# zhu-xlab/PFST

Measured on AMD Instinct MI355X. Metric: PFST train-step images/s on 1024² IRRG tiles, higher is better.
Workload: dtype f32 (f16x3 split MFMA: two scaled fp16 pieces per operand, three products, fp32 accumulate); 1 GPU; pfst_pots_irrg2vaih_irrg_deeplabv3plus_r50-d8; global_batch=8, per_gpu_batch=8, tile=1024x1024x3, num_classes=6, parallelism=dp1, weights=seeded random init, conv_math=f16x3

## Files before the change

### pfst_amd/csrc/conv_epilogue.h

```cpp
#pragma once
#include <type_traits>
#include <utility>
#include "common.h"
#ifndef PFST_BNB_LOAD_AUX
#define PFST_BNB_LOAD_AUX 0
#endif
#include "../../include/pfst_hip.h"

typedef float pfst_f32x16 __attribute__((ext_vector_type(16)));

__device__ __forceinline__ bool src_coord(int o, int t, int a, int b, int c0, int div, int lim, int& s) {
  const int v = o * a + t * b + c0;
  const int odd = v & (div - 1);
  s = v >> (div >> 1);
  return (odd == 0) & (s >= 0) & (s < lim);
}

template <int... Is, class F>
__device__ __forceinline__ void static_for_seq(std::integer_sequence<int, Is...>, F&& f) {
  (f(std::integral_constant<int, Is>()), ...);
}
template <int N, class F>
__device__ __forceinline__ void static_for(F&& f) {
  static_for_seq(std::make_integer_sequence<int, N>(), static_cast<F&&>(f));
}

typedef pfst_bnb_fuse_t PfstBnbArgs;

template <int CTRL>
__device__ __forceinline__ float lane_xchg(float v) {
  if (CTRL == 0) return __builtin_bit_cast(float, __builtin_amdgcn_ds_swizzle(__builtin_bit_cast(int, v), 0x401F));
  return __builtin_bit_cast(float, __builtin_amdgcn_update_dpp(0, __builtin_bit_cast(int, v), CTRL, 0xF, 0xF, true));
}
template <int OP>
__device__ __forceinline__ float lane_combine(float a, float b) {
  return OP == 0 ? a + b : (OP == 1 ? fminf(a, b) : fmaxf(a, b));
}
template <int H, int CTRL, int OP = 0>
__device__ __forceinline__ void butterfly_step(float* a, bool upper) {
#pragma unroll
  for (int k = 0; k < H; ++k) {
    const float send = upper ? a[k] : a[k + H];
    const float keep = upper ? a[k + H] : a[k];
    a[k] = lane_combine<OP>(keep, lane_xchg<CTRL>(send));
  }
}
template <int NV, int OP = 0>
__device__ __forceinline__ float half_wave_transpose_reduce(float (&a)[NV], int l31) {
  static_assert(NV == 32 || NV == 16, "one value per accumulator row of a 64- or 32-row wave tile");
  if (NV == 32) {
    butterfly_step<16, 0, OP>(a, (l31 & 16) != 0);
  } else {
#pragma unroll
    for (int k = 0; k < 16; ++k) a[k] = lane_combine<OP>(a[k], lane_xchg<0>(a[k]));
  }
  butterfly_step<8, 0x140, OP>(a, (l31 & 8) != 0);
  butterfly_step<4, 0x141, OP>(a, (l31 & 4) != 0);
  butterfly_step<2, 0x4E, OP>(a, (l31 & 2) != 0);
  butterfly_step<1, 0xB1, OP>(a, (l31 & 1) != 0);
  return a[0];
}
template <int NV>
__device__ __forceinline__ float half_wave_transpose_sum(float (&a)[NV], int l31) { return half_wave_transpose_reduce<NV, 0>(a, l31); }

constexpr int PFST_ROWSUM_LDS_FLOATS = 64 * 20;
__device__ __forceinline__ void wave_lds_phase_fence() {
  __builtin_amdgcn_fence(__ATOMIC_RELEASE, "wavefront");
  __builtin_amdgcn_wave_barrier();
  __builtin_amdgcn_fence(__ATOMIC_ACQUIRE, "wavefront");
}

__device__ __forceinline__ float half_wave_rowsum_lds(const float (&v)[16], float* __restrict__ ws, int lane) {
  float4* wr = reinterpret_cast<float4*>(ws + lane * 20);
  wave_lds_phase_fence();
  wr[0] = make_float4(v[0], v[1], v[2], v[3]);
  wr[1] = make_float4(v[4], v[5], v[6], v[7]);
  wr[2] = make_float4(v[8], v[9], v[10], v[11]);
  wr[3] = make_float4(v[12], v[13], v[14], v[15]);
  wave_lds_phase_fence();
  const int l31 = lane & 31;
  const float* rd = ws + ((lane & 32) + (l31 >> 4)) * 20 + (l31 & 15);
  float s = 0.f;
#pragma unroll
  for (int i = 0; i < 16; ++i) s += rd[i * 40];
  return s + lane_xchg<0>(s);
}

template <int TM, int TN, int WAVES_N, int BN, int BNB = 0, bool LDSRED = false>
__device__ __forceinline__ void conv_epilogue(pfst_f32x16 (&acc)[TM][TN], float* __restrict__ out, const float* __restrict__ bias,
                                              float* __restrict__ stats, int stats_T, int accumulate, int M, int P, int m0, int p0,
                                              int wm0, int wn0, int bx, int n, int wid, int lane, const PfstBnbArgs& bnb = PfstBnbArgs(),
                                              float* __restrict__ lds = nullptr, const float* __restrict__ gsrc = nullptr,
                                              const unsigned long long* __restrict__ gmask = nullptr, float* __restrict__ stats_mm = nullptr,
                                              bool nt_store = false) {
  const int l31 = lane & 31, lh = lane >> 5;
  if (BNB == 0 && stats) {
    const int gx = (P + BN - 1) / BN;
    const int slot = (n * gx + bx) * WAVES_N + (wid % WAVES_N);
    if constexpr (LDSRED) {
      float* ws = lds + wid * PFST_ROWSUM_LDS_FLOATS;
#pragma unroll
      for (int i = 0; i < TM; ++i) {
        float sv[16], sq[16];
#pragma unroll
        for (int r = 0; r < 16; ++r) {
          float a = 0.f, b = 0.f;
#pragma unroll
          for (int j = 0; j < TN; ++j) {
            const int pp = p0 + wn0 + j * 32 + l31;
            const float v = pp < P ? acc[i][j][r] : 0.f;
            a += v;
            b = fmaf(v, v, b);
          }
          sv[r] = a;
          sq[r] = b;
        }
        const float ts = half_wave_rowsum_lds(sv, ws, lane);
        const float tq = half_wave_rowsum_lds(sq, ws, lane);
        const int r = l31 & 15;
        const int m = m0 + wm0 + i * 32 + (r & 3) + 8 * (r >> 2) + 4 * lh;
        if (l31 < 16 && m < M) reinterpret_cast<float2*>(stats)[(i64)m * stats_T + slot] = make_float2(ts, tq);
      }
    } else {
    constexpr int NV = TM * 16;
    float sv[NV], sq[NV];
#pragma unroll
    for (int i = 0; i < TM; ++i) {
#pragma unroll
      for (int r = 0; r < 16; ++r) {
        float a = 0.f, b = 0.f;
#pragma unroll
        for (int j = 0; j < TN; ++j) {
          const int pp = p0 + wn0 + j * 32 + l31;
          const float v = pp < P ? acc[i][j][r] : 0.f;
          a += v;
          b = fmaf(v, v, b);
        }
        sv[i * 16 + r] = a;
        sq[i * 16 + r] = b;
      }
    }
    const float ts = half_wave_transpose_sum<NV>(sv, l31);
    const float tq = half_wave_transpose_sum<NV>(sq, l31);
    const int e = l31 & (NV - 1), r = e & 15;
    const int m = m0 + wm0 + (e >> 4) * 32 + (r & 3) + 8 * (r >> 2) + 4 * lh;
    if (l31 < NV && m < M) {
      float2* dst = reinterpret_cast<float2*>(stats) + ((i64)m * stats_T + slot);
      *dst = make_float2(ts, tq);
    }
    if (stats_mm) {
      const float inf = __builtin_inff();
#pragma unroll
      for (int i = 0; i < TM; ++i) {
#pragma unroll
        for (int rr = 0; rr < 16; ++rr) {
          float lo = inf, hi = -inf;
#pragma unroll
          for (int j = 0; j < TN; ++j) {
            const int pp = p0 + wn0 + j * 32 + l31;
            const float v = acc[i][j][rr];
            lo = pp < P ? fminf(lo, v) : lo;
            hi = pp < P ? fmaxf(hi, v) : hi;
          }
          sv[i * 16 + rr] = lo;
          sq[i * 16 + rr] = hi;
        }
      }
      const float tlo = half_wave_transpose_reduce<NV, 1>(sv, l31);
      const float thi = half_wave_transpose_reduce<NV, 2>(sq, l31);
      if (l31 < NV && m < M) reinterpret_cast<float2*>(stats_mm)[(i64)m * stats_T + slot] = make_float2(tlo, thi);
    }
    }
  }
  if (BNB != 0 || (!bias && m0 + wm0 + TM * 32 <= M)) {
    constexpr unsigned OOB = 0x80000000u;
    const __amdgpu_buffer_rsrc_t rsrc = __builtin_amdgcn_make_buffer_rsrc(out, 0, M * P * 4, 0x00020000);
    unsigned voff[TN];
#pragma unroll
    for (int j = 0; j < TN; ++j) {
      const int pp = p0 + wn0 + j * 32 + l31;
      voff[j] = pp < P ? 4u * ((unsigned)pp + 4u * (unsigned)lh * (unsigned)P) : OOB;
    }
    const int row0 = m0 + wm0;
    const bool gated = gsrc != nullptr;
    static_assert(TN <= 2, "the gate words are shared by the column blocks of a 64-pixel wave tile");
    const __amdgpu_buffer_rsrc_t grs = __builtin_amdgcn_make_buffer_rsrc(const_cast<float*>(gated ? gsrc : out), 0, M * P * 4, 0x00020000);
    const __amdgpu_buffer_rsrc_t mrs =
        __builtin_amdgcn_make_buffer_rsrc(const_cast<unsigned long long*>(gmask), 0, gated ? M * (P >> 6) * 8 : 0, 0x00020000);
    const int gpp = p0 + wn0 + l31, gbit = (gpp & 255) >> 2;
    const unsigned mvoff = 8u * (unsigned)((gpp >> 8) * 4 + (gpp & 3)) + 4u * (unsigned)(gbit >> 5) + 32u * (unsigned)lh * (unsigned)(P >> 6);
    auto load_gate = [&](int i, int (&gw)[16]) {
#pragma unroll
      for (int r = 0; r < 16; ++r)
        gw[r] = gated ? __builtin_amdgcn_raw_buffer_load_b32(mrs, mvoff, 8 * (P >> 6) * (row0 + i * 32 + (r & 3) + 8 * (r >> 2)), 0) : 0;
    };
    auto load_addend = [&](int i, int j, const int (&gw)[16], float (&old)[16]) {
#pragma unroll
      for (int r = 0; r < 16; ++r)
        old[r] = __builtin_bit_cast(float, __builtin_amdgcn_raw_buffer_load_b32(grs, voff[j], 4 * P * (row0 + i * 32 + (r & 3) + 8 * (r >> 2)), 0));
      if (gated) {
        const unsigned sh = (unsigned)((gbit & 31) + 8 * j);
#pragma unroll
        for (int r = 0; r < 16; ++r)
          old[r] = __builtin_bit_cast(float, __builtin_bit_cast(int, old[r]) & __builtin_amdgcn_sbfe(gw[r], sh, 1u));
      }
    };
    if (BNB && (accumulate || gated)) {
#pragma unroll
      for (int i = 0; i < TM; ++i) {
        int gw[16];
        load_gate(i, gw);
#pragma unroll
        for (int j = 0; j < TN; ++j) {
          float old[16];
          load_addend(i, j, gw, old);
#pragma unroll
          for (int r = 0; r < 16; ++r) acc[i][j][r] += old[r];
        }
      }
    }
    if (BNB || !(accumulate || gated)) {
      auto store_all = [&](auto aux_c) {
        constexpr int AUX = decltype(aux_c)::value;
#pragma unroll
        for (int i = 0; i < TM; ++i)
#pragma unroll
          for (int j = 0; j < TN; ++j) {
#pragma unroll
            for (int r = 0; r < 16; ++r) {
              const float v = acc[i][j][r];
#ifdef PFST_DIAG_NO_STORE
              if (v != 1.2345e-30f) continue;
#endif
              __builtin_amdgcn_raw_buffer_store_b32(__builtin_bit_cast(unsigned, v), rsrc, voff[j],
                                                    4 * P * (row0 + i * 32 + (r & 3) + 8 * (r >> 2)), AUX);
            }
          }
      };
#ifdef PFST_BNB_NT_STORE
      if (nt_store) store_all(std::integral_constant<int, 2>());
#else
      if (BNB == 0 && nt_store) store_all(std::integral_constant<int, 2>());
#endif
      else store_all(std::integral_constant<int, 0>());
    } else {
#pragma unroll
      for (int i = 0; i < TM; ++i) {
        int gw[16];
        load_gate(i, gw);
#pragma unroll
        for (int j = 0; j < TN; ++j) {
          float old[16];
          load_addend(i, j, gw, old);
#pragma unroll
          for (int r = 0; r < 16; ++r)
          {
            const float v = acc[i][j][r] + old[r];
            __builtin_amdgcn_raw_buffer_store_b32(__builtin_bit_cast(unsigned, v), rsrc, voff[j],
                                                  4 * P * (row0 + i * 32 + (r & 3) + 8 * (r >> 2)), 0);
          }
        }
      }
    }
    if (BNB) {
      const __amdgpu_buffer_rsrc_t xr = __builtin_amdgcn_make_buffer_rsrc(const_cast<float*>(bnb.x) + (i64)n * bnb.x_bs, 0, M * P * 4, 0x00020000);
      const __amdgpu_buffer_rsrc_t yr = __builtin_amdgcn_make_buffer_rsrc(const_cast<float*>(bnb.y ? bnb.y + (i64)n * bnb.y_bs : bnb.x), 0,
                                                                          M * P * 4, 0x00020000);
      const __amdgpu_buffer_rsrc_t cr = __builtin_amdgcn_make_buffer_rsrc(const_cast<float*>(bnb.coef), 0, M * 16, 0x00020000);
      constexpr bool gate_x = BNB == 1, gate_y = BNB == 2, gate_m = BNB == 4;
      const __amdgpu_buffer_rsrc_t ymr = __builtin_amdgcn_make_buffer_rsrc(
          const_cast<unsigned long long*>(gate_m ? bnb.y_mask + (i64)n * M * (P >> 6) : nullptr), 0, gate_m ? M * (P >> 6) * 8 : 0, 0x00020000);
      const unsigned cvoff = 64u * (unsigned)lh + 8u;
      const int gxp = (P + BN - 1) / BN;
      const int slot = (n * gxp + bx) * WAVES_N + (wid % WAVES_N);
#pragma unroll
      for (int i = 0; i < TM; ++i) {
        float sv[16], sq[16];
        int yw[gate_m ? 16 : 1];
        if constexpr (gate_m) {
#pragma unroll
          for (int r = 0; r < 16; ++r)
            yw[r] = __builtin_amdgcn_raw_buffer_load_b32(ymr, mvoff, 8 * (P >> 6) * (row0 + i * 32 + (r & 3) + 8 * (r >> 2)), 0);
        }
#pragma unroll
        for (int r = 0; r < 16; ++r) {
          const int row = row0 + i * 32 + (r & 3) + 8 * (r >> 2);
          float sc = 0.f, sh = 0.f;
          if (gate_x) {
            const float2 c2 = __builtin_bit_cast(float2, __builtin_amdgcn_raw_buffer_load_b64(cr, cvoff, 16 * row, 0));
            sc = c2.x; sh = c2.y;
          }
          float a = 0.f, b = 0.f;
#pragma unroll
          for (int j = 0; j < TN; ++j) {
            const float xv = __builtin_bit_cast(float, __builtin_amdgcn_raw_buffer_load_b32(xr, voff[j], 4 * P * row, PFST_BNB_LOAD_AUX));
            float dz = voff[j] != OOB ? acc[i][j][r] : 0.f;
            if (gate_y) {
              const float yv = __builtin_bit_cast(float, __builtin_amdgcn_raw_buffer_load_b32(yr, voff[j], 4 * P * row, PFST_BNB_LOAD_AUX));
              dz = yv > 0.f ? dz : 0.f;
            } else if (gate_x) {
              dz = __fmaf_rn(xv, sc, sh) > 0.f ? dz : 0.f;
            } else if constexpr (gate_m) {
              dz = __builtin_bit_cast(float, __builtin_bit_cast(int, dz) & __builtin_amdgcn_sbfe(yw[r], (unsigned)((gbit & 31) + 8 * j), 1u));
            }
            a += dz;
            b = fmaf(dz, xv, b);
          }
          sv[r] = a;
          sq[r] = b;
          if ((r & 3) == 3) __builtin_amdgcn_sched_barrier(0);
        }
        float* ws = lds + wid * PFST_ROWSUM_LDS_FLOATS;
        const float ts = LDSRED ? half_wave_rowsum_lds(sv, ws, lane) : half_wave_transpose_sum<16>(sv, l31);
        const float tq = LDSRED ? half_wave_rowsum_lds(sq, ws, lane) : half_wave_transpose_sum<16>(sq, l31);
        const int r = l31 & 15;
        const int m = row0 + i * 32 + (r & 3) + 8 * (r >> 2) + 4 * lh;
        if (l31 < 16) reinterpret_cast<float2*>(bnb.partials)[(i64)m * stats_T + slot] = make_float2(ts, tq);
      }
    }
    return;
  }
#pragma unroll
  for (int i = 0; i < TM; ++i) {
#pragma unroll
    for (int j = 0; j < TN; ++j) {
      const int pp = p0 + wn0 + j * 32 + l31;
#pragma unroll
      for (int r = 0; r < 16; ++r) {
        const int m = m0 + wm0 + i * 32 + (r & 3) + 8 * (r >> 2) + 4 * lh;
        if (m < M && pp < P) {
          float v = acc[i][j][r];
          if (bias) v += bias[m];
          const i64 idx = (i64)m * P + pp;
          if (accumulate) v += out[idx];
          out[idx] = v;
        }
      }
    }
  }
}
```

### pfst_amd/csrc/conv_f16x3.hip

```cpp
#include "conv_epilogue.h"
#include "amax.h"
#include "wgrad_launch.h"
#include "weight_jobs.h"
#include <math.h>
#include <stdlib.h>
#include <type_traits>
#include <utility>
#include "../../include/pfst_hip.h"

typedef _Float16 f16x8 __attribute__((ext_vector_type(8)));
typedef float f32x4 __attribute__((ext_vector_type(4)));

namespace {

constexpr int BN = 128;
constexpr int NP = 2;

__global__ __launch_bounds__(256) void absmax_kernel(const float* __restrict__ x, i64 n, i64 plane_stride, int slot_stride,
                                                     float* __restrict__ slots) {
  const float* p = x + (i64)blockIdx.y * plane_stride;
  float m = 0.f;
  const i64 n4 = (((uintptr_t)p & 15) == 0) ? n / 4 : 0;
  for (i64 i = (i64)blockIdx.x * blockDim.x + threadIdx.x; i < n4; i += (i64)gridDim.x * blockDim.x) {
    const float4 v = reinterpret_cast<const float4*>(p)[i];
// ... 269 lines not shown
        voff2 = tap_voff(0);
      } else {
        voff2 = OOB;
      }
    }
  };

  const int eb = amax_exponent(amax_read(in_amax));
  const float sb = __builtin_bit_cast(float, __builtin_amdgcn_readfirstlane(__builtin_bit_cast(int, scale_of(eb))));
  int ea = 0, ea_y = -1;

  auto prologue = [&](int lin) {
    ld_lin = lin;
    set_load_side(lin);
    tap2 = sidx2 = 0;
    voff2 = tap_voff(0);
    static_for<8 * TPT>([&](auto vc) { load_b(vc, std::integral_constant<int, 0>(), voff2, 0); });
    static_for<NA>([&](auto vc) { load_a(vc, std::integral_constant<int, 0>(), 0); });
    advance();
#pragma unroll
    for (int v = 0; v < NA; ++v) As[(v / (NA / 2)) * TILE_A + tid + NT * (v % (NA / 2))] = areg[0][v];
#pragma unroll
    for (int t = 0; t < TPT; ++t) {
      uint4 ph, pl;
      if constexpr (BNL) {
        const float2* cf = reinterpret_cast<const float2*>(bnl_s) + (t + bt) * 16 + kh * 8;
#pragma unroll
        for (int i = 0; i < 8; ++i) breg[0][t][i] = fmaxf(__fmaf_rn(breg[0][t][i], cf[i].x, cf[i].y), 0.f);
      }
      if constexpr (BPACK) unpack8_f16(breg[0][t], ph, pl);
      else split8_f16(breg[0][t], sb, ph, pl);
      Bs[(t + bt) * TILE_B + (0 * 2 + kh) * BN + pix] = ph;
      Bs[(t + bt) * TILE_B + (1 * 2 + kh) * BN + pix] = pl;
    }
    {
      const int soff = sidx2 * chan_step, a_soff = (tap2 * spt + sidx2) * 2 * a_tile;
      static_for<8 * TPT>([&](auto vc) { load_b(vc, std::integral_constant<int, 1>(), voff2, soff); });
      static_for<NA>([&](auto vc) { load_a(vc, std::integral_constant<int, 1>(), a_soff); });
    }
    advance();
    __syncthreads();
  };

  const int l15 = lane & 15, lq = lane >> 4;
  const int a_frag = (lq >> 1) * TILE_A + (lq & 1) * BM + wm0 + l15;
  const int b_frag = (lq >> 1) * TILE_B + (lq & 1) * BN + wn0 + l15;

  const int l31 = lane & 31, lh = lane >> 5;
  auto step32 = [&](auto setn_c, int k) {
    constexpr int SETN = decltype(setn_c)::value, SETL = SETN ^ 1;
    constexpr int CUR = SETL * PAIR_CHUNKS, NXT = SETN * PAIR_CHUNKS;
    f16x8 af[2][TMW][NP], bf[2][2][NP];
    auto rd_a = [&](int t, int i, int pl) { af[t][i][pl] = __builtin_bit_cast(f16x8, As[CUR + t * TILE_A + (pl * 2 + lh) * BM + wm0 + i * 32 + l31]); };
    auto rd_b = [&](int t, int j, int pl) { bf[t][j][pl] = __builtin_bit_cast(f16x8, Bs[CUR + t * TILE_B + (pl * 2 + lh) * BN + wn0 + j * 32 + l31]); };
    constexpr int RG = 2 + TMW;
    auto read_frag = [&](auto rc) {
      constexpr int r = decltype(rc)::value, grp = r / RG, e = r % RG, t = grp & 1, pa = grp < 2 ? 1 : 0, pb = grp < 2 ? 0 : 1;
      if constexpr (e == 0) rd_a(t, 0, pa);
      else if constexpr (e == 1) rd_b(t, 0, pb);
      else if constexpr (e == 2) rd_b(t, 1, pb);
      else rd_a(t, 1, pa);
    };
    const int soff2 = sidx2 * chan_step;
    const int a_soff2 = (tap2 * spt + sidx2) * 2 * a_tile;
    constexpr int PRE = TMW == 2 ? RG : 2 * RG;
    static_for<PRE>([&](auto rc) { read_frag(rc); });
    __builtin_amdgcn_sched_barrier(0);
    SplitF16 s0, s1;
    uint4 cfr[BNL ? 4 : 1];
    const int cf_at = BNL ? sidx1 * 16 + bt * 8 + kh * 4 : 0;
    auto filler = [&](auto sc) {
      constexpr int m = decltype(sc)::value;
      if constexpr (m < 8) {
        if constexpr (TPT == 2) {
          load_b(std::integral_constant<int, 2 * m>(), std::integral_constant<int, SETL>(), voff2, soff2);
          load_b(std::integral_constant<int, 2 * m + 1>(), std::integral_constant<int, SETL>(), voff2, soff2);
        } else {
          load_b(std::integral_constant<int, m>(), std::integral_constant<int, SETL>(), voff2, soff2);
        }
      }
      if constexpr (m >= 8 && m < 8 + NA) As[NXT + ((m - 8) / (NA / 2)) * TILE_A + tid + NT * ((m - 8) % (NA / 2))] = areg[SETN][m - 8];
      if constexpr (BNL && m >= 8 && m < 12) cfr[m - 8] = bnl_s[cf_at + (m - 8)];
      if constexpr (m >= 12) {
        constexpr int SPS = 2 * TPT;
        static_for<SPS>([&](auto kc) {
          constexpr int kk = (m - 12) * SPS + decltype(kc)::value;
          if constexpr (BPACK) {
            if constexpr (kk < 8) unpack_op_f16<kk>(breg[SETN][0], s0);
            else if constexpr (kk < 16 && TPT == 2) unpack_op_f16<kk - 8>(breg[SETN][TPT - 1], s1);
          } else {
            if constexpr (BNL && kk < 24 && kk % 6 < 2) {
              constexpr int e = 2 * (kk / 6) + kk % 6;
              const uint4 c2 = cfr[e >> 1];
              const float sc = __builtin_bit_cast(float, (e & 1) ? c2.z : c2.x), sh = __builtin_bit_cast(float, (e & 1) ? c2.w : c2.y);
              breg[SETN][0][e] = fmaxf(__fmaf_rn(breg[SETN][0][e], sc, sh), 0.f);
            }
            if constexpr (kk < 24) split_op_f16<kk>(breg[SETN][0], sb, s0);
            else split_op_f16<kk - 24>(breg[SETN][TPT - 1], sb, s1);
          }
        });
      }
      if constexpr (m >= 12 && m < 12 + NA) load_a(std::integral_constant<int, m - 12>(), std::integral_constant<int, SETL>(), a_soff2);
      if constexpr (m == 18 && TPT == 2) {
        Bs[NXT + (0 * 2 + kh) * BN + pix] = make_uint4(s0.h[0], s0.h[1], s0.h[2], s0.h[3]);
        Bs[NXT + (1 * 2 + kh) * BN + pix] = make_uint4(s0.l[0], s0.l[1], s0.l[2], s0.l[3]);
      }
      if constexpr (m == 23 && TPT == 2) {
        Bs[NXT + TILE_B + (0 * 2 + kh) * BN + pix] = make_uint4(s1.h[0], s1.h[1], s1.h[2], s1.h[3]);
        Bs[NXT + TILE_B + (1 * 2 + kh) * BN + pix] = make_uint4(s1.l[0], s1.l[1], s1.l[2], s1.l[3]);
      }
      if constexpr (m == 23 && TPT == 1) {
        Bs[NXT + bt * TILE_B + (0 * 2 + kh) * BN + pix] = make_uint4(s0.h[0], s0.h[1], s0.h[2], s0.h[3]);
        Bs[NXT + bt * TILE_B + (1 * 2 + kh) * BN + pix] = make_uint4(s0.l[0], s0.l[1], s0.l[2], s0.l[3]);
      }
    };
    static_for<12 * TMW>([&](auto mc) {
      constexpr int m = decltype(mc)::value;
      constexpr int prod = m / (4 * TMW), rem = m % (4 * TMW), t = rem / (2 * TMW), i = (rem >> 1) % TMW, j = rem & 1;
      constexpr int pa = prod == 0 ? 1 : 0, pb = prod == 1 ? 1 : 0;
      acc32[i][j] = __builtin_amdgcn_mfma_f32_32x32x16_f16(af[t][i][pa], bf[t][j][pb], acc32[i][j], 0, 0, 0);
      if constexpr (PRE + m < 4 * RG) read_frag(std::integral_constant<int, PRE + m>());
      if constexpr (TMW == 2) {
        filler(std::integral_constant<int, m>());
      } else {
        filler(std::integral_constant<int, 2 * m>());
        filler(std::integral_constant<int, 2 * m + 1>());
      }
      __builtin_amdgcn_sched_barrier(0);
    });
    advance();
    __syncthreads();
  };
  auto epilogue = [&](int lin) {
    int bx, by, y, n;
    decode(lin, bx, by, y, n);
    if (y != ea_y) {
      ea = amax_exponent(amax_read(w_amax + (i64)y * PFST_AMAX_SUB));
      ea_y = y;
    }
    const int p0 = bx * BN, m0 = by * BM;
    float* const outn = out + (i64)n * out_bs;
    const float* const gsrc = gate.g ? gate.g + (i64)n * gate.g_bs : nullptr;
    const unsigned long long* const gmask = gate.g ? gate.mask + (i64)n * M * (P >> 6) : nullptr;
    const float ua = unscale_of(ea), ub = unscale_of(eb);
    {
#pragma unroll
      for (int i = 0; i < TMW; ++i)
#pragma unroll
        for (int j = 0; j < 2; ++j)
#pragma unroll
          for (int r = 0; r < 16; ++r) acc32[i][j][r] = acc32[i][j][r] * ua * ub;
      if constexpr (BNB != 0) {
        static_assert(PAIR_CHUNKS * sizeof(uint4) >= (NT / 64) * PFST_ROWSUM_LDS_FLOATS * sizeof(float), "epilogue scratch must fit into one pair buffer");
        conv_epilogue<2, 2, WAVES_N, BN, BNB, true>(acc32, outn, bias, stats, stats_T, accumulate, M, P, m0, p0, wm0, wn0, bx, n, wid, lane, bnb,
                                                    reinterpret_cast<float*>(smem + PAIR_CHUNKS), gsrc, gmask, nullptr, nt_out);
        __syncthreads();
      } else {
#ifdef PFST_STATS_LDSRED
        if (stats && !stats_mm && BMT != 64) {
          conv_epilogue<TMW, 2, WAVES_N, BN, 0, true>(acc32, outn, bias, stats, stats_T, accumulate, M, P, m0, p0, wm0, wn0, bx, n, wid, lane, PfstBnbArgs(),
                                                      reinterpret_cast<float*>(smem + PAIR_CHUNKS), gsrc, gmask, nullptr, nt_out);
          __syncthreads();
        } else
#endif
        conv_epilogue<TMW, 2, WAVES_N, BN>(acc32, outn, bias, stats, stats_T, accumulate, M, P, m0, p0, wm0, wn0, bx, n, wid, lane, PfstBnbArgs(), nullptr,
                                           gsrc, gmask, stats_mm, nt_out);
      }
#pragma unroll
      for (int i = 0; i < TMW; ++i)
#pragma unroll
        for (int j = 0; j < 2; ++j)
#pragma unroll
          for (int r = 0; r < 16; ++r) acc32[i][j][r] = 0.f;
    }
  };

  for (int lin = blockIdx.x; lin < total; lin += G) {
    if (!CHAIN || lin == (int)blockIdx.x) prologue(lin);
    for (int k = 0; k < KP; k += 2) {
      step32(std::integral_constant<int, 1>(), k);
      if (k + 1 < KP) step32(std::integral_constant<int, 0>(), k + 1);
    }
    epilogue(lin);
  }
}

template <int SHAPE, bool BPACK = false, bool ONE = false, int BMT = 128>
__global__ __launch_bounds__(BMT == 64 ? 256 : 2 * BMT, BMT == 256 ? 1 : 2) void conv_igemm_f16x3_kernel(
    const float* __restrict__ in, i64 in_bs, const uint4* __restrict__ wk4, const float* __restrict__ bias,
    float* __restrict__ out, i64 out_bs, int C, int Hi, int Wi, int M, int Ho, int Wo, int ks,
    int ca, int cb, int cc, int cdivv, int accumulate, float* __restrict__ stats, int stats_T,
    const float* __restrict__ w_amax, const float* __restrict__ in_amax, int Y, int Z, int chain, PfstResGate gate) {
  conv_igemm_f16x3_body<SHAPE, 0, BPACK, ONE, BMT>(in, in_bs, wk4, bias, out, out_bs, C, Hi, Wi, M, Ho, Wo, ks, ca, cb, cc, cdivv, accumulate, stats, stats_T,
                               w_amax, in_amax, Y, Z, chain, PfstBnbArgs(), gate);
}
__global__ __launch_bounds__(512, 1) void conv_igemm_f16x3_bnl_kernel(
    const float* __restrict__ in, i64 in_bs, const uint4* __restrict__ wk4, const float* __restrict__ bias,
    float* __restrict__ out, i64 out_bs, int C, int Hi, int Wi, int M, int Ho, int Wo, int ks,
    int ca, int cb, int cc, int cdivv, int accumulate, float* __restrict__ stats, int stats_T,
    const float* __restrict__ w_amax, const float* __restrict__ in_amax, int Y, int Z, int chain, const float4* __restrict__ bnl) {
  conv_igemm_f16x3_body<32, 0, false, true, 256, true>(in, in_bs, wk4, bias, out, out_bs, C, Hi, Wi, M, Ho, Wo, ks, ca, cb, cc, cdivv, accumulate, stats,
                                                       stats_T, w_amax, in_amax, Y, Z, chain, PfstBnbArgs(), PfstResGate(), bnl);
}
template <int BNB, bool ONE = false, int BMT = 128>
__global__ __launch_bounds__(2 * BMT, BMT == 128 ? 2 : 1) void conv_igemm_f16x3_bnb_kernel(
    const float* __restrict__ in, i64 in_bs, const uint4* __restrict__ wk4, const float* __restrict__ bias,
    float* __restrict__ out, i64 out_bs, int C, int Hi, int Wi, int M, int Ho, int Wo, int ks,
    int ca, int cb, int cc, int cdivv, int accumulate, float* __restrict__ stats, int stats_T,
    const float* __restrict__ w_amax, const float* __restrict__ in_amax, int Y, int Z, int chain, PfstBnbArgs bnb, PfstResGate gate) {
  conv_igemm_f16x3_body<32, BNB, false, ONE, BMT>(in, in_bs, wk4, bias, out, out_bs, C, Hi, Wi, M, Ho, Wo, ks, ca, cb, cc, cdivv, accumulate, stats, stats_T,
                                 w_amax, in_amax, Y, Z, chain, bnb, gate);
}


typedef float f32x16 __attribute__((ext_vector_type(16)));

struct Split4 {
  unsigned h[2], l[2];
  float t0[2], t1[2];
};
#ifdef PFST_F16X3_SPLIT6
template <int K>
__device__ __forceinline__ void split4_op_f16(const float (&v)[4], float s, Split4& st) {
  constexpr int q = K / 6, op = K % 6;
  if constexpr (op == 0) asm volatile("v_mul_f32 %0, %1, %2" : "=v"(st.t0[q]) : "s"(s), "v"(v[2 * q]));
  else if constexpr (op == 1) asm volatile("v_mul_f32 %0, %1, %2" : "=v"(st.t1[q]) : "s"(s), "v"(v[2 * q + 1]));
  else if constexpr (op == 2) asm volatile("v_cvt_pk_f16_f32 %0, %1, %2" : "=v"(st.h[q]) : "v"(st.t0[q]), "v"(st.t1[q]));
  else if constexpr (op == 3)
    asm volatile("v_fma_mix_f32 %0, %1, %2, -%3 op_sel:[0,0,0] op_sel_hi:[0,0,1]" : "=v"(st.t0[q]) : "v"(v[2 * q]), "s"(s), "v"(st.h[q]));
  else if constexpr (op == 4)
    asm volatile("v_fma_mix_f32 %0, %1, %2, -%3 op_sel:[0,0,1] op_sel_hi:[0,0,1]" : "=v"(st.t1[q]) : "v"(v[2 * q + 1]), "s"(s), "v"(st.h[q]));
  else asm volatile("v_cvt_pk_f16_f32 %0, %1, %2" : "=v"(st.l[q]) : "v"(st.t0[q]), "v"(st.t1[q]));
}
#else
template <int K>
__device__ __forceinline__ void split4_op_f16(const float (&v)[4], float s, Split4& st) {
  constexpr int q = K / 6, op = K % 6;
  if constexpr (op == 2) asm volatile("v_fma_mixlo_f16 %0, %1, %2, 0 op_sel_hi:[0,0,0]" : "=v"(st.h[q]) : "v"(v[2 * q]), "s"(s));
  else if constexpr (op == 3) asm volatile("v_fma_mixhi_f16 %0, %1, %2, 0 op_sel_hi:[0,0,0]" : "+v"(st.h[q]) : "v"(v[2 * q + 1]), "s"(s));
  else if constexpr (op == 4)
    asm volatile("v_fma_mixlo_f16 %0, %1, %2, -%3 op_sel:[0,0,0] op_sel_hi:[0,0,1]" : "=v"(st.l[q]) : "v"(v[2 * q]), "s"(s), "v"(st.h[q]));
  else if constexpr (op == 5)
    asm volatile("v_fma_mixhi_f16 %0, %1, %2, -%3 op_sel:[0,0,1] op_sel_hi:[0,0,1]" : "+v"(st.l[q]) : "v"(v[2 * q + 1]), "s"(s), "v"(st.h[q]));
}
#endif
template <int K>
__device__ __forceinline__ void unpack4_op_f16(const float (&v)[4], Split4& st) {
  constexpr int q = K & 1;
  if constexpr (K < 2) asm volatile("v_perm_b32 %0, %1, %2, %3" : "=v"(st.h[q]) : "v"(v[2 * q + 1]), "v"(v[2 * q]), "s"(0x05040100u));
  else asm volatile("v_perm_b32 %0, %1, %2, %3" : "=v"(st.l[q]) : "v"(v[2 * q + 1]), "v"(v[2 * q]), "s"(0x07060302u));
}

template <bool PACK, int BMT = 128, bool BNL = false>
__global__ __launch_bounds__(2 * BMT, BMT == 128 ? 2 : 1) void conv_wgrad_f16x3_line_kernel(
    const float* __restrict__ x, i64 x_bs, const float* __restrict__ dy, i64 dy_bs, float* __restrict__ dw,
    int J, int M, int P, int chunks, int chunk_len, int N, i64 x_gs, i64 dy_gs, i64 dw_gs, int gx, int gy, int gz,
    const float* __restrict__ x_amax, const float* __restrict__ dy_amax, const float4* __restrict__ bnl) {
  static_assert(!BNL || !PACK, "a pre-split operand is already normalised");
  constexpr int BM = BMT, BJ = 128, WM = 64, WAVES_N = 2, WN = 64, TM = 2, TN = 2, NT = 2 * BM;
  constexpr int RPP = NT / 8;
  constexpr int PA = BM / RPP, PB = BJ / RPP;
  constexpr int ROWS_A = BM + 2, ROWS_B = BJ + 2;
  constexpr int TILE_A = 4 * ROWS_A + 4, TILE_B = 4 * ROWS_B + 4;
  __shared__ uint4 As[2][2 * TILE_A];
  __shared__ uint4 Bs[2][2 * TILE_B];

  const int tid = threadIdx.x, lane = tid & 63, wid = __builtin_amdgcn_readfirstlane(tid >> 6);
  const int wm0 = (wid / WAVES_N) * WM, wn0 = (wid % WAVES_N) * WN;
  int bx, by, bz;
  {
    const int lin = blockIdx.x, tiles = gx * gy, z8 = gz & ~7;
    if (lin < tiles * z8) {
      const int xcd = lin & 7, idx = lin >> 3;
      const int sl = idx / tiles, t = idx - sl * tiles;
      bz = sl * 8 + xcd;
      by = t / gx;
      bx = t - by * gx;
    } else {
      bz = lin / tiles;
      const int t = lin - bz * tiles;
      by = t / gx;
      bx = t - by * gx;
    }
  }
  const int j0 = bx * BJ, m0 = by * BM;
  const int ng = bz / chunks, chunk = bz - ng * chunks;
  const int grp = ng / N, n = ng - grp * N;
  const int pbeg = chunk * chunk_len;
  const int pend = min(P, pbeg + chunk_len);
  if (pbeg >= pend) return;
  x += (i64)grp * x_gs + (i64)n * x_bs;
  dy += (i64)grp * dy_gs + (i64)n * dy_bs;
  dw += dw_gs >= 0 ? (i64)grp * dw_gs : (i64)bz * -dw_gs;
  const int ea = amax_exponent(amax_read(dy_amax)), eb = amax_exponent(amax_read(x_amax));
  const float sa = __builtin_bit_cast(float, __builtin_amdgcn_readfirstlane(__builtin_bit_cast(int, scale_of(ea))));
  const float sb = __builtin_bit_cast(float, __builtin_amdgcn_readfirstlane(__builtin_bit_cast(int, scale_of(eb))));
  const __amdgpu_buffer_rsrc_t a_rsrc = __builtin_amdgcn_make_buffer_rsrc(const_cast<float*>(dy), 0, M * P * 4, 0x00020000);
  const __amdgpu_buffer_rsrc_t b_rsrc = __builtin_amdgcn_make_buffer_rsrc(const_cast<float*>(x), 0, J * P * 4, 0x00020000);

  const int rslot = tid >> 3, seg = tid & 7;
  constexpr unsigned OOB = 0x80000000u;
  const unsigned a_voff = 4u * ((unsigned)(m0 + rslot) * (unsigned)P) + 16u * seg;
  const unsigned b_voff = 4u * ((unsigned)(j0 + rslot) * (unsigned)P) + 16u * seg;
  const int row_step = RPP * P * 4;
  const int a_half = 2 * ((seg >> 2) * TILE_A + ((seg >> 1) & 1) * ROWS_A + rslot) + (seg & 1);
  const int b_half = 2 * ((seg >> 2) * TILE_B + ((seg >> 1) & 1) * ROWS_B + rslot) + (seg & 1);

  float la[2][PA][4], lb[2][PB][4];
  float bsc[BNL ? PB : 1], bsh[BNL ? PB : 1];
  if constexpr (BNL) {
#pragma unroll
    for (int p = 0; p < PB; ++p) {
      const int j = j0 + rslot + p * RPP;
      const float4 cf = j < J ? bnl[j] : make_float4(0.f, 0.f, 0.f, 0.f);
      bsc[p] = cf.z;
      bsh[p] = cf.w;
    }
  }
// ... 367 lines not shown
```

Before: 29.57 images/s.

## Software-pipeline epilogue addend and BN-backward input loads with double buffering

Restructures the conv epilogue so the global loads of the residual/gate addend blocks and of the BN-backward x/y/coef/mask operands are issued one block ahead, into double-buffered registers, with sched_barriers fencing each stage. This hides global-load latency behind the arithmetic and stores of the previous block instead of serialising load-then-use per row. It also enlarges the row group from 4 to 8 rows in pipelined mode. The cost is higher register pressure from the double buffers, which could reduce occupancy or cause spills in the MFMA kernel.

```diff
diff --git a/pfst_amd/csrc/conv_epilogue.h b/pfst_amd/csrc/conv_epilogue.h
--- a/pfst_amd/csrc/conv_epilogue.h
+++ b/pfst_amd/csrc/conv_epilogue.h
@@ -86,7 +86,7 @@
   return s + lane_xchg<0>(s);
 }
 
-template <int TM, int TN, int WAVES_N, int BN, int BNB = 0, bool LDSRED = false>
+template <int TM, int TN, int WAVES_N, int BN, int BNB = 0, bool LDSRED = false, bool PIPE = false>
 __device__ __forceinline__ void conv_epilogue(pfst_f32x16 (&acc)[TM][TN], float* __restrict__ out, const float* __restrict__ bias,
                                               float* __restrict__ stats, int stats_T, int accumulate, int M, int P, int m0, int p0,
                                               int wm0, int wn0, int bx, int n, int wid, int lane, const PfstBnbArgs& bnb = PfstBnbArgs(),
@@ -189,35 +189,84 @@
         __builtin_amdgcn_make_buffer_rsrc(const_cast<unsigned long long*>(gmask), 0, gated ? M * (P >> 6) * 8 : 0, 0x00020000);
     const int gpp = p0 + wn0 + l31, gbit = (gpp & 255) >> 2;
     const unsigned mvoff = 8u * (unsigned)((gpp >> 8) * 4 + (gpp & 3)) + 4u * (unsigned)(gbit >> 5) + 32u * (unsigned)lh * (unsigned)(P >> 6);
-    auto load_gate = [&](int i, int (&gw)[16]) {
-#pragma unroll
-      for (int r = 0; r < 16; ++r)
-        gw[r] = gated ? __builtin_amdgcn_raw_buffer_load_b32(mrs, mvoff, 8 * (P >> 6) * (row0 + i * 32 + (r & 3) + 8 * (r >> 2)), 0) : 0;
+    auto addend_pipeline = [&](auto gated_c) {
+      constexpr bool GATED = decltype(gated_c)::value;
+      constexpr int NB = TM * TN;
+      int gw[2][GATED ? 16 : 1];
+      float old[2][16];
+      auto issue = [&](auto bc) {
+        constexpr int b = decltype(bc)::value, i = b / TN, j = b % TN;
+        if constexpr (GATED && j == 0) {
+#pragma unroll
+          for (int r = 0; r < 16; ++r)
+            gw[i & 1][r] = __builtin_amdgcn_raw_buffer_load_b32(mrs, mvoff, 8 * (P >> 6) * (row0 + i * 32 + (r & 3) + 8 * (r >> 2)), 0);
+        }
+#pragma unroll
+        for (int r = 0; r < 16; ++r)
+          old[b & 1][r] =
+              __builtin_bit_cast(float, __builtin_amdgcn_raw_buffer_load_b32(grs, voff[j], 4 * P * (row0 + i * 32 + (r & 3) + 8 * (r >> 2)), 0));
+      };
+      if constexpr (PIPE) issue(std::integral_constant<int, 0>());
+      static_for<NB>([&](auto bc) {
+        constexpr int b = decltype(bc)::value, i = b / TN, j = b % TN;
+        if constexpr (!PIPE) issue(bc);
+        else if constexpr (b + 1 < NB) issue(std::integral_constant<int, b + 1>());
+        __builtin_amdgcn_sched_barrier(0);
+        if constexpr (GATED) {
+          const unsigned sh = (unsigned)((gbit & 31) + 8 * j);
+#pragma unroll
+          for (int r = 0; r < 16; ++r)
+            old[b & 1][r] = __builtin_bit_cast(float, __builtin_bit_cast(int, old[b & 1][r]) & __builtin_amdgcn_sbfe(gw[i & 1][r], sh, 1u));
+        }
+        if constexpr (BNB != 0) {
+#pragma unroll
+          for (int r = 0; r < 16; ++r) acc[i][j][r] += old[b & 1][r];
+        } else {
+#pragma unroll
+          for (int r = 0; r < 16; ++r) {
+            const float v = acc[i][j][r] + old[b & 1][r];
+            __builtin_amdgcn_raw_buffer_store_b32(__builtin_bit_cast(unsigned, v), rsrc, voff[j],
+                                                  4 * P * (row0 + i * 32 + (r & 3) + 8 * (r >> 2)), 0);
+          }
+        }
+        __builtin_amdgcn_sched_barrier(0);
+      });
     };
-    auto load_addend = [&](int i, int j, const int (&gw)[16], float (&old)[16]) {
-#pragma unroll
-      for (int r = 0; r < 16; ++r)
-        old[r] = __builtin_bit_cast(float, __builtin_amdgcn_raw_buffer_load_b32(grs, voff[j], 4 * P * (row0 + i * 32 + (r & 3) + 8 * (r >> 2)), 0));
-      if (gated) {
-        const unsigned sh = (unsigned)((gbit & 31) + 8 * j);
-#pragma unroll
-        for (int r = 0; r < 16; ++r)
-          old[r] = __builtin_bit_cast(float, __builtin_bit_cast(int, old[r]) & __builtin_amdgcn_sbfe(gw[r], sh, 1u));
+    if (accumulate || gated) {
+      if (gated) addend_pipeline(std::true_type());
+      else addend_pipeline(std::false_type());
+    }
+    constexpr bool gate_x = BNB == 1, gate_y = BNB == 2, gate_m = BNB == 4;
+    constexpr int SG = PIPE ? 8 : 4, NG = TM * 16 / SG;
+    const __amdgpu_buffer_rsrc_t xr =
+        __builtin_amdgcn_make_buffer_rsrc(const_cast<float*>(BNB != 0 ? bnb.x + (i64)n * bnb.x_bs : nullptr), 0, M * P * 4, 0x00020000);
+    const __amdgpu_buffer_rsrc_t yr = __builtin_amdgcn_make_buffer_rsrc(const_cast<float*>(BNB != 0 && bnb.y ? bnb.y + (i64)n * bnb.y_bs : bnb.x), 0,
+                                                                        M * P * 4, 0x00020000);
+    const __amdgpu_buffer_rsrc_t cr = __builtin_amdgcn_make_buffer_rsrc(const_cast<float*>(bnb.coef), 0, M * 16, 0x00020000);
+    const __amdgpu_buffer_rsrc_t ymr = __builtin_amdgcn_make_buffer_rsrc(
+        const_cast<unsigned long long*>(gate_m ? bnb.y_mask + (i64)n * M * (P >> 6) : nullptr), 0, gate_m ? M * (P >> 6) * 8 : 0, 0x00020000);
+    const unsigned cvoff = 64u * (unsigned)lh + 8u;
+    float xs[2][SG][TN], ys[2][gate_y ? SG : 1][TN];
+    float2 cs[2][gate_x ? SG : 1];
+    int yws[2][gate_m ? SG : 1];
+    auto sums_issue = [&](auto gc) {
+      constexpr int g = decltype(gc)::value, i = g * SG / 16, r0 = g * SG % 16;
+#pragma unroll
+      for (int rr = 0; rr < SG; ++rr) {
+        const int r = r0 + rr, row = row0 + i * 32 + (r & 3) + 8 * (r >> 2);
+        if constexpr (gate_x) cs[g & 1][rr] = __builtin_bit_cast(float2, __builtin_amdgcn_raw_buffer_load_b64(cr, cvoff, 16 * row, 0));
+        if constexpr (gate_m) yws[g & 1][rr] = __builtin_amdgcn_raw_buffer_load_b32(ymr, mvoff, 8 * (P >> 6) * row, 0);
+#pragma unroll
+        for (int j = 0; j < TN; ++j) {
+          xs[g & 1][rr][j] = __builtin_bit_cast(float, __builtin_amdgcn_raw_buffer_load_b32(xr, voff[j], 4 * P * row, PFST_BNB_LOAD_AUX));
+          if constexpr (gate_y)
+            ys[g & 1][rr][j] = __builtin_bit_cast(float, __builtin_amdgcn_raw_buffer_load_b32(yr, voff[j], 4 * P * row, PFST_BNB_LOAD_AUX));
+        }
       }
     };
-    if (BNB && (accumulate || gated)) {
-#pragma unroll
-      for (int i = 0; i < TM; ++i) {
-        int gw[16];
-        load_gate(i, gw);
-#pragma unroll
-        for (int j = 0; j < TN; ++j) {
-          float old[16];
-          load_addend(i, j, gw, old);
-#pragma unroll
-          for (int r = 0; r < 16; ++r) acc[i][j][r] += old[r];
-        }
-      }
+    if constexpr (BNB != 0 && PIPE) {
+      sums_issue(std::integral_constant<int, 0>());
+      __builtin_amdgcn_sched_barrier(0);
     }
     if (BNB || !(accumulate || gated)) {
       auto store_all = [&](auto aux_c) {
@@ -243,80 +292,47 @@
       if (BNB == 0 && nt_store) store_all(std::integral_constant<int, 2>());
 #endif
       else store_all(std::integral_constant<int, 0>());
-    } else {
-#pragma unroll
-      for (int i = 0; i < TM; ++i) {
-        int gw[16];
-        load_gate(i, gw);
-#pragma unroll
-        for (int j = 0; j < TN; ++j) {
-          float old[16];
-          load_addend(i, j, gw, old);
-#pragma unroll
-          for (int r = 0; r < 16; ++r)
-          {
-            const float v = acc[i][j][r] + old[r];
-            __builtin_amdgcn_raw_buffer_store_b32(__builtin_bit_cast(unsigned, v), rsrc, voff[j],
-                                                  4 * P * (row0 + i * 32 + (r & 3) + 8 * (r >> 2)), 0);
-          }
-        }
-      }
-    }
-    if (BNB) {
-      const __amdgpu_buffer_rsrc_t xr = __builtin_amdgcn_make_buffer_rsrc(const_cast<float*>(bnb.x) + (i64)n * bnb.x_bs, 0, M * P * 4, 0x00020000);
-      const __amdgpu_buffer_rsrc_t yr = __builtin_amdgcn_make_buffer_rsrc(const_cast<float*>(bnb.y ? bnb.y + (i64)n * bnb.y_bs : bnb.x), 0,
-                                                                          M * P * 4, 0x00020000);
-      const __amdgpu_buffer_rsrc_t cr = __builtin_amdgcn_make_buffer_rsrc(const_cast<float*>(bnb.coef), 0, M * 16, 0x00020000);
-      constexpr bool gate_x = BNB == 1, gate_y = BNB == 2, gate_m = BNB == 4;
-      const __amdgpu_buffer_rsrc_t ymr = __builtin_amdgcn_make_buffer_rsrc(
-          const_cast<unsigned long long*>(gate_m ? bnb.y_mask + (i64)n * M * (P >> 6) : nullptr), 0, gate_m ? M * (P >> 6) * 8 : 0, 0x00020000);
-      const unsigned cvoff = 64u * (unsigned)lh + 8u;
+    }
+    if constexpr (BNB != 0) {
       const int gxp = (P + BN - 1) / BN;
       const int slot = (n * gxp + bx) * WAVES_N + (wid % WAVES_N);
-#pragma unroll
-      for (int i = 0; i < TM; ++i) {
-        float sv[16], sq[16];
-        int yw[gate_m ? 16 : 1];
-        if constexpr (gate_m) {
-#pragma unroll
-          for (int r = 0; r < 16; ++r)
-            yw[r] = __builtin_amdgcn_raw_buffer_load_b32(ymr, mvoff, 8 * (P >> 6) * (row0 + i * 32 + (r & 3) + 8 * (r >> 2)), 0);
-        }
-#pragma unroll
-        for (int r = 0; r < 16; ++r) {
-          const int row = row0 + i * 32 + (r & 3) + 8 * (r >> 2);
-          float sc = 0.f, sh = 0.f;
-          if (gate_x) {
-            const float2 c2 = __builtin_bit_cast(float2, __builtin_amdgcn_raw_buffer_load_b64(cr, cvoff, 16 * row, 0));
-            sc = c2.x; sh = c2.y;
-          }
+      float sv[16], sq[16];
+      static_for<NG>([&](auto gc) {
+        constexpr int g = decltype(gc)::value, i = g * SG / 16, r0 = g * SG % 16;
+        if constexpr (!PIPE) sums_issue(gc);
+        else if constexpr (g + 1 < NG) sums_issue(std::integral_constant<int, g + 1>());
+        __builtin_amdgcn_sched_barrier(0);
+#pragma unroll
+        for (int rr = 0; rr < SG; ++rr) {
+          const int r = r0 + rr;
           float a = 0.f, b = 0.f;
 #pragma unroll
           for (int j = 0; j < TN; ++j) {
-            const float xv = __builtin_bit_cast(float, __builtin_amdgcn_raw_buffer_load_b32(xr, voff[j], 4 * P * row, PFST_BNB_LOAD_AUX));
+            const float xv = xs[g & 1][rr][j];
             float dz = voff[j] != OOB ? acc[i][j][r] : 0.f;
-            if (gate_y) {
-              const float yv = __builtin_bit_cast(float, __builtin_amdgcn_raw_buffer_load_b32(yr, voff[j], 4 * P * row, PFST_BNB_LOAD_AUX));
-              dz = yv > 0.f ? dz : 0.f;
-            } else if (gate_x) {
-              dz = __fmaf_rn(xv, sc, sh) > 0.f ? dz : 0.f;
+            if constexpr (gate_y) {
+              dz = ys[g & 1][rr][j] > 0.f ? dz : 0.f;
+            } else if constexpr (gate_x) {
+              dz = __fmaf_rn(xv, cs[g & 1][rr].x, cs[g & 1][rr].y) > 0.f ? dz : 0.f;
             } else if constexpr (gate_m) {
-              dz = __builtin_bit_cast(float, __builtin_bit_cast(int, dz) & __builtin_amdgcn_sbfe(yw[r], (unsigned)((gbit & 31) + 8 * j), 1u));
+              dz = __builtin_bit_cast(float, __builtin_bit_cast(int, dz) & __builtin_amdgcn_sbfe(yws[g & 1][rr], (unsigned)((gbit & 31) + 8 * j), 1u));
             }
             a += dz;
             b = fmaf(dz, xv, b);
           }
           sv[r] = a;
           sq[r] = b;
-          if ((r & 3) == 3) __builtin_amdgcn_sched_barrier(0);
-        }
-        float* ws = lds + wid * PFST_ROWSUM_LDS_FLOATS;
-        const float ts = LDSRED ? half_wave_rowsum_lds(sv, ws, lane) : half_wave_transpose_sum<16>(sv, l31);
-        const float tq = LDSRED ? half_wave_rowsum_lds(sq, ws, lane) : half_wave_transpose_sum<16>(sq, l31);
-        const int r = l31 & 15;
-        const int m = row0 + i * 32 + (r & 3) + 8 * (r >> 2) + 4 * lh;
-        if (l31 < 16) reinterpret_cast<float2*>(bnb.partials)[(i64)m * stats_T + slot] = make_float2(ts, tq);
-      }
+        }
+        if constexpr (r0 + SG == 16) {
+          float* ws = lds + wid * PFST_ROWSUM_LDS_FLOATS;
+          const float ts = LDSRED ? half_wave_rowsum_lds(sv, ws, lane) : half_wave_transpose_sum<16>(sv, l31);
+          const float tq = LDSRED ? half_wave_rowsum_lds(sq, ws, lane) : half_wave_transpose_sum<16>(sq, l31);
+          const int r = l31 & 15;
+          const int m = row0 + i * 32 + (r & 3) + 8 * (r >> 2) + 4 * lh;
+          if (l31 < 16) reinterpret_cast<float2*>(bnb.partials)[(i64)m * stats_T + slot] = make_float2(ts, tq);
+        }
+        __builtin_amdgcn_sched_barrier(0);
+      });
     }
     return;
   }
diff --git a/pfst_amd/csrc/conv_f16x3.hip b/pfst_amd/csrc/conv_f16x3.hip
--- a/pfst_amd/csrc/conv_f16x3.hip
+++ b/pfst_amd/csrc/conv_f16x3.hip
@@ -445,18 +445,18 @@
           for (int r = 0; r < 16; ++r) acc32[i][j][r] = acc32[i][j][r] * ua * ub;
       if constexpr (BNB != 0) {
         static_assert(PAIR_CHUNKS * sizeof(uint4) >= (NT / 64) * PFST_ROWSUM_LDS_FLOATS * sizeof(float), "epilogue scratch must fit into one pair buffer");
-        conv_epilogue<2, 2, WAVES_N, BN, BNB, true>(acc32, outn, bias, stats, stats_T, accumulate, M, P, m0, p0, wm0, wn0, bx, n, wid, lane, bnb,
+        conv_epilogue<2, 2, WAVES_N, BN, BNB, true, true>(acc32, outn, bias, stats, stats_T, accumulate, M, P, m0, p0, wm0, wn0, bx, n, wid, lane, bnb,
                                                     reinterpret_cast<float*>(smem + PAIR_CHUNKS), gsrc, gmask, nullptr, nt_out);
         __syncthreads();
       } else {
 #ifdef PFST_STATS_LDSRED
         if (stats && !stats_mm && BMT != 64) {
-          conv_epilogue<TMW, 2, WAVES_N, BN, 0, true>(acc32, outn, bias, stats, stats_T, accumulate, M, P, m0, p0, wm0, wn0, bx, n, wid, lane, PfstBnbArgs(),
+          conv_epilogue<TMW, 2, WAVES_N, BN, 0, true, true>(acc32, outn, bias, stats, stats_T, accumulate, M, P, m0, p0, wm0, wn0, bx, n, wid, lane, PfstBnbArgs(),
                                                       reinterpret_cast<float*>(smem + PAIR_CHUNKS), gsrc, gmask, nullptr, nt_out);
           __syncthreads();
         } else
 #endif
-        conv_epilogue<TMW, 2, WAVES_N, BN>(acc32, outn, bias, stats, stats_T, accumulate, M, P, m0, p0, wm0, wn0, bx, n, wid, lane, PfstBnbArgs(), nullptr,
+        conv_epilogue<TMW, 2, WAVES_N, BN, 0, false, true>(acc32, outn, bias, stats, stats_T, accumulate, M, P, m0, p0, wm0, wn0, bx, n, wid, lane, PfstBnbArgs(), nullptr,
                                            gsrc, gmask, stats_mm, nt_out);
       }
 #pragma unroll
```

Result: no change. 29.68 images/s, median of 6 (+0.4%).
